# FalkorDB/FalkorDB

Measured on AMD Instinct MI355X. Metric: traversed edges/sec (TEPS) on k-hop MATCH, RMAT scale-22/26; % HBM roofline, higher is better.
Workload: dtype u32

## Files before the change

falkordb_amd/csrc/bitexpand.hip:

```cpp
#include "bitexpand.hpp"

namespace fgpu {

constexpr u32 BP_ITEM = 256;
static_assert(BP_ITEM == 256, "bp_pull_kernel<.., SPARSE> unrolls an item into four 64-entry trips");
constexpr u32 BP_VCHUNK = 4096;

static fgpu_info bp_acc_alloc(fgpu_ctx* ctx, DevBuf<u64>& acc) {
    FGPU_TRY(acc.alloc(ctx, BP_ACC_WORDS));
    FGPU_HIP(hipMemsetAsync(acc.p, 0, BP_ACC_WORDS * sizeof(u64), ctx->stream()));
    return FGPU_OK;
}
__global__ __launch_bounds__(256) void bp_acc_fold_kernel(unsigned long long* __restrict__ acc, u32* __restrict__ pub, u32 seq) {
    __shared__ u64 s_a[4], s_b[4];
    u64 a = acc[(size_t)threadIdx.x * BP_ACC_STRIDE], b = acc[(size_t)threadIdx.x * BP_ACC_STRIDE + 1];
#pragma unroll
    for (int d = 32; d >= 1; d >>= 1) { a += __shfl_xor(a, d, 64); b += __shfl_xor(b, d, 64); }
    if (lane_id() == 0) { s_a[threadIdx.x >> 6] = a; s_b[threadIdx.x >> 6] = b; }
    __syncthreads();
    if (threadIdx.x == 0) {
        const u64 sa = s_a[0] + s_a[1] + s_a[2] + s_a[3], sb = s_b[0] + s_b[1] + s_b[2] + s_b[3];
        if (pub) {
            __hip_atomic_store(pub + 0, (u32)sa, __ATOMIC_RELAXED, __HIP_MEMORY_SCOPE_SYSTEM);
            __hip_atomic_store(pub + 1, (u32)(sa >> 32), __ATOMIC_RELAXED, __HIP_MEMORY_SCOPE_SYSTEM);
// ... 1640 lines not shown
}

static fgpu_info bp_count_finish(fgpu_ctx* ctx, BitState& s, u32 n_out, u32 ntouched, const HopOut& out, u64* nnz, u64* checksum) {
    if (ntouched) {
        ProfScope ps(ctx, "bp_count_kernel<side rows>", (u64)ntouched * s.w * 8);
        DevBuf<u32> vmap;
        FGPU_TRY(vmap.alloc(ctx, (size_t)ntouched + 1));
        FGPU_TRY(launch(bp_slot_vertex_kernel, dim3(ctx->cus * 4), dim3(256), 0, ctx->stream(), out.fin.tbits, out.fin.tpref, n_out, vmap.p));
        FGPU_TRY(bp_count_rows(ctx, s, out.y, ntouched, out.fin.label, out.fin.tab, (u64*)out.fin.acc, 16, vmap.p));
    }
    FGPU_TRY(bp_acc_read(ctx, (u64*)out.fin.acc, nnz, checksum));
    bp_recycle_state(ctx, s);
    s.n = n_out;
    return FGPU_OK;
}

fgpu_info bp_hop(fgpu_ctx* ctx, BitState& s, const fgpu_mat* m, const fgpu_mat* dp, const fgpu_mat* dm, u64* flops,
                 const fgpu_mat* next_m, const fgpu_mat* count_next) {
    HopPlan p;
    FGPU_TRY(bp_hop_enter(ctx, s, m, dp, flops, false));
    FGPU_TRY(bp_hop_plan(ctx, s, m, dp, dm, 0, next_m, count_next, p));
    BitState o;
    bp_layout(o, (u32)m->ncols, s.nsrc);
    FGPU_TRY(bp_alloc_zero(ctx, o.x, o));
    FGPU_TRY(bp_alloc_flags(ctx, o));
    const HopOut out = {o.x.p, o.flag.p, BpFinal{nullptr, nullptr, nullptr, nullptr, nullptr, 0}};
    FusedStats st;
    int pull_idx = -1;
    if (p.t) FGPU_TRY(bp_pull(ctx, p, s, out, next_m, &st, &pull_idx));
    FGPU_TRY(bp_delta_fixups(ctx, p, s, out));
    return bp_hop_finish(ctx, p, s, o, next_m, st, pull_idx);
}

__global__ __launch_bounds__(256) void bp_hub_check_kernel(const u64* __restrict__ x, u32 slot, u32 ws, u32 nsrc, const u32* __restrict__ rowmap,
                                                           const u64* __restrict__ rowhash, u64* __restrict__ out) {
    __shared__ u64 s_h[4];
    bool bad = false;
    for (u32 k = threadIdx.x; k < ws; k += 256) {
        const u32 lo = k * 64;
        const u64 want = nsrc >= lo + 64 ? ~0ull : nsrc > lo ? (1ull << (nsrc - lo)) - 1ull : 0ull;
        bad |= x[(size_t)slot * ws + k] != want;
    }
    u64 hs = 0;
    for (u32 i = threadIdx.x; i < nsrc; i += 256) hs += rowhash ? rowhash[i] : cs_row_hash(rowmap ? (u64)rowmap[i] : (u64)i);
#pragma unroll
    for (int d = 32; d >= 1; d >>= 1) hs += (u64)__shfl_xor((long long)hs, d, 64);
    if (lane_id() == 0) s_h[threadIdx.x >> 6] = hs;
    const int nbad = __syncthreads_count(bad ? 1 : 0);
    if (threadIdx.x == 0) {
        out[0] = nbad == 0 && nsrc ? 1ull : 0ull;
        out[1] = s_h[0] + s_h[1] + s_h[2] + s_h[3];
    }
}
__global__ __launch_bounds__(256) void bp_hub_sums_kernel(const u32* __restrict__ rows, u32 deg, u64 dsum, const u64* __restrict__ label,
                                                          u32 nsrc, const u64* __restrict__ hsum, int with_sum,
                                                          unsigned long long* __restrict__ acc) {
    u64 cnt = 0, ds = 0;
    if (!label) {
        if (blockIdx.x == 0 && threadIdx.x == 0) { cnt = deg; ds = dsum; }
    } else {
        for (u32 i = blockIdx.x * 256 + threadIdx.x; i < deg; i += gridDim.x * 256) {
            const u32 v = rows[i];
            if ((label[v >> 6] >> (v & 63u)) & 1ull) { ++cnt; ds += cs_dest_hash(v); }
        }
    }
    bp_block_add2(cnt * nsrc, with_sum ? ds * hsum[0] : 0ull, acc);
}
static fgpu_info bp_hub_rows(fgpu_ctx* ctx, const BitState& s, const BpXPlan* xp, int mode, const u64* label_dev, u64* acc,
                             const BpXPlan** hub) {
    *hub = nullptr;
    BpXHub hb;
    if (!bp_xplan_hub(xp, &hb) || hb.slot >= s.n || !s.nsrc) return FGPU_OK;
    DevBuf<u64> chk;
    FGPU_TRY(chk.alloc(ctx, 2));
    FGPU_TRY(launch(bp_hub_check_kernel, dim3(1), dim3(256), 0, ctx->stream(), (const u64*)s.x.p, hb.slot, s.ws, s.nsrc,
                    (const u32*)s.rowmap.p, (const u64*)s.rowhash.p, chk.p));
    u32 sat = 0;
    FGPU_TRY(read_u32(ctx, (const u32*)chk.p, &sat));
    if (!sat) return FGPU_OK;
    ProfScope ps(ctx, "xp_hub_rows", (u64)hb.deg * (label_dev ? 4 : 0));
    u32 grid = label_dev ? cdiv(hb.deg, 256) : 1u;
    if (grid > (u32)ctx->cus * 4) grid = ctx->cus * 4;
    FGPU_TRY(launch(bp_hub_sums_kernel, dim3(grid), dim3(256), 0, ctx->stream(), hb.rows, hb.deg, hb.dsum, label_dev, s.nsrc,
                    (const u64*)(chk.p + 1), mode == 2 ? 1 : 0, (unsigned long long*)acc));
    *hub = hb.plan;
    return FGPU_OK;
}

fgpu_info bp_hop_count(fgpu_ctx* ctx, BitState& s, const fgpu_mat* m, const fgpu_mat* dp, const fgpu_mat* dm, u64* flops,
                       const u64* label_dev, u64* nnz, u64* checksum) {
    HopPlan p;
    FGPU_TRY(bp_hop_enter(ctx, s, m, dp, flops, true));
    FGPU_TRY(bp_hop_plan(ctx, s, m, dp, dm, checksum ? 2 : 1, nullptr, nullptr, p));
    FGPU_TRY(bp_relayout(ctx, s, bp_xplan_perm(p.xp)));
    const u32 n_out = (u32)m->ncols;
    DevBuf<u64> tbits, side, tab, acc;
    DevBuf<u32> tpref;
    u32 ntouched = 0;
    if (!p.no_touched) FGPU_TRY(bp_touched_side(ctx, p, s, n_out, tbits, tpref, side, &ntouched));
    FGPU_TRY(bp_acc_alloc(ctx, acc));
    if (p.mode == 2) FGPU_TRY(bp_cs_tables(ctx, s, tab));
    const HopOut out = {side.p, nullptr, BpFinal{tbits.p, tpref.p, label_dev, tab.p, (unsigned long long*)acc.p, s.w}};
    const u64 xrows = s.nz_rows < (u64)s.n ? s.nz_rows : (u64)s.n;
    const BpXPlan* hub = nullptr;
    if (p.no_touched) FGPU_TRY(bp_hub_rows(ctx, s, p.xp, p.mode, label_dev, acc.p, &hub));
    if (p.xp) FGPU_TRY(bp_xpull_count(ctx, hub ? hub : p.xp, p.t, s.x.p, s.ws, p.mode, out.fin, side.p, p.lds_tables, xrows));
    else if (p.t) FGPU_TRY(bp_pull(ctx, p, s, out, nullptr, nullptr, nullptr));
    FGPU_TRY(bp_delta_fixups(ctx, p, s, out));
    return bp_count_finish(ctx, s, n_out, ntouched, out, nnz, checksum);
}

fgpu_info bp_count_hub_in(fgpu_ctx* ctx, const fgpu_mat* m, u32 nsrc, const u64** in_bits) {
    *in_bits = nullptr;
    BitState lay;
    bp_layout(lay, (u32)m->nrows, nsrc);
    if (!m->nnz || m->is_hyper() || !bp_xcd_applies(ctx, lay.n, lay.ws)) return FGPU_OK;
    const fgpu_mat* t = nullptr;
    const BpXPlan* xp = nullptr;
    BpXHub hb;
    FGPU_TRY(transposed_with_items(ctx, m, &t));
    FGPU_TRY(bp_xplan(ctx, m, t, &xp));
    if (bp_xplan_hub(xp, &hb)) *in_bits = hb.in_bits;
    return FGPU_OK;
}

__global__ __launch_bounds__(256) void bp_probe_rows_kernel(CsrView at, const u32* __restrict__ dst, const u32* __restrict__ bit, u32 k,
                                                            const u64* __restrict__ x, u32 ws, uint8_t* __restrict__ hit) {
    const u32 lane = lane_id();
    const u32 wave = (blockIdx.x * 256 + threadIdx.x) >> 6, nwaves = (gridDim.x * 256) >> 6;
    for (u32 i = wave; i < k; i += nwaves) {
        const u32 v = dst[i], j = bit[i];
        if (v == 0xFFFFFFFFu || j == 0xFFFFFFFFu) continue;
        u32 b, e;
        row_range(at, v, b, e);
        bool found = false;
        for (u32 q0 = b; q0 < e && !found; q0 += 64) {
            const u32 q = q0 + lane;
            bool h = false;
            if (q < e) h = (x[(size_t)at.colidx[q] * ws + (j >> 6)] >> (j & 63)) & 1ull;
            found = __ballot(h) != 0ull;
        }
        if (found && lane == 0) hit[i] = 1;
    }
}
__global__ __launch_bounds__(256) void bp_probe_delta_kernel(CsrView d, u32 nnz, const u32* __restrict__ wordrow,
                                                             const u32* __restrict__ sdst, const u32* __restrict__ srow, u32 k,
                                                             const u32* __restrict__ bit, const u64* __restrict__ x, u32 ws,
                                                             uint8_t* __restrict__ hit) {
    for (u32 q = blockIdx.x * 256 + threadIdx.x; q < nnz; q += gridDim.x * 256) {
        const u32 v = d.colidx[q];
        u32 lo = 0, hi = k;
        while (lo < hi) {
            const u32 mid = (lo + hi) >> 1;
            if (sdst[mid] < v) lo = mid + 1; else hi = mid;
        }
// ... 335 lines not shown
```

falkordb_amd/csrc/bitexpand.hpp:

```cpp
#pragma once
#include "common.hpp"

namespace fgpu {

constexpr u32 BP_ACC_SLOTS = 256, BP_ACC_STRIDE = 16;
constexpr size_t BP_ACC_WORDS = (size_t)BP_ACC_SLOTS * BP_ACC_STRIDE;
__device__ __forceinline__ void bp_block_add2(u64 a, u64 b, unsigned long long* __restrict__ acc) {
    __shared__ u64 s_acc_red[32];
#pragma unroll
    for (int d = 32; d >= 1; d >>= 1) {
        a += __shfl_xor(a, d, 64);
        b += __shfl_xor(b, d, 64);
    }
    const u32 wv = threadIdx.x >> 6, nw = (blockDim.x + 63) >> 6;
    if (lane_id() == 0) { s_acc_red[wv] = a; s_acc_red[16 + wv] = b; }
    __syncthreads();
    if (threadIdx.x == 0) {
        u64 sa = 0, sb = 0;
        for (u32 i = 0; i < nw; ++i) { sa += s_acc_red[i]; sb += s_acc_red[16 + i]; }
        unsigned long long* slot = acc + (size_t)(blockIdx.x % BP_ACC_SLOTS) * BP_ACC_STRIDE;
        if (sa) atomicAdd(slot, (unsigned long long)sa);
        if (sb) atomicAdd(slot + 1, (unsigned long long)sb);
    }
}

struct BpFinal {
    const u64* tbits;
    const u32* tpref;
    const u64* label;
    const u64* tab;
    unsigned long long* acc;
    u32 w;
};

struct BpXPlan;
fgpu_info bp_xplan(fgpu_ctx* ctx, const fgpu_mat* m, const fgpu_mat* t, const BpXPlan** out);
fgpu_info bp_xplan_chunks(fgpu_ctx* ctx, const BpXPlan* xp, uint32_t** out, uint64_t* nwords);
const u32* bp_xplan_perm(const BpXPlan* p);
struct BpXHub {
    const BpXPlan* plan;
    u32 slot;
    u32 deg;
    u64 dsum;
    const u32* rows;
    const u64* in_bits;
};
bool bp_xplan_hub(const BpXPlan* xp, BpXHub* out);
fgpu_info bp_xpull_count(fgpu_ctx* ctx, const BpXPlan* xp, const fgpu_mat* t, const u64* x, u32 ws, int mode, const BpFinal& fin,
                         u64* side, size_t lds_tables, u64 xrows);
bool bp_xfold_fits(const fgpu_ctx* ctx, u32 ws, int mode, size_t lds_tables);

}
```

falkordb_amd/csrc/bitpart.hip:

```cpp
#include "bitexpand.hpp"

namespace fgpu {

constexpr u32 XP_FIRST = 0x80000000u;
constexpr u32 XP_SPAN = 768;
constexpr u32 XP_RUNW = 8;
constexpr int XP_FOLD_THREADS = 512;
constexpr u32 XP_RUNS = XP_SPAN / XP_RUNW;
constexpr u32 XP_NO_VTX = 0xFFFFFFFFu;

struct BpXPlan {
    bool usable = false;
    u32 n = 0, ng = 0;
    int cut = 0;
    int dense = 0;
    u32 nd = 0;
    DevBuf<u32> gvtx;
    u64 nentries = 0;
    u32 nprows = 0;
    u32 nchunks = 0;
    DevBuf<u32> pcol;
    u32 pstart[9] = {0, 0, 0, 0, 0, 0, 0, 0, 0};
    u32 cbase[9] = {0, 0, 0, 0, 0, 0, 0, 0, 0};
    DevBuf<u32> pstart_dev;
    DevBuf<u32> cstart;
    DevBuf<u32> crun0;
    DevBuf<uint8_t> cshared;
    DevBuf<u32> zrows;
    u32 nzrows = 0;
    DevBuf<u64> ne;
    DevBuf<u32> pbase;
    int direct = 0;
    u64 ndirect = 0;
    DevBuf<u64> de;
    DevBuf<u32> dbase;
    DevBuf<u32> dcol;
    DevBuf<u32> perm;
    BpXPlanPtr hub;
    u32 hub_v = 0, hub_slot = 0;
    u32 hub_deg = 0;
    u64 hub_dsum = 0;
    DevBuf<u32> hub_rows;
    DevBuf<u64> hub_in;
    const BpXPlan* full = nullptr;
};
const u32* bp_xplan_perm(const BpXPlan* p) { return p ? p->perm.p : nullptr; }
void BpXPlanDelete::operator()(BpXPlan* p) const { delete p; }

__global__ __launch_bounds__(256) void xp_runs_kernel(const uint2* __restrict__ pairs, const u32* __restrict__ pstart, u32 n, u32 nnz,
                                                      u32* __restrict__ pcol, u32* __restrict__ off) {
    __shared__ u32 s_ps[9];
    if (threadIdx.x < 9) s_ps[threadIdx.x] = pstart[threadIdx.x];
    __syncthreads();
    const u32 lane = lane_id();
    const u32 wave = (blockIdx.x * 256 + threadIdx.x) >> 6, nwaves = (gridDim.x * 256) >> 6;
    for (u32 p0 = wave * 64; p0 < nnz; p0 += nwaves * 64) {
        const u32 p = p0 + lane;
        u32 g0 = 0, g1 = 0;
        size_t base = 0;
        if (p < nnz) {
            u32 x = 0;
#pragma unroll
            for (u32 k = 1; k < 8; ++k) x += p >= s_ps[k] ? 1u : 0u;
            const uint2 e = pairs[p];
            const bool head = p == s_ps[x];
            const u32 prev = head ? 0xFFFFFFFFu : pairs[p - 1].y;
            const bool first = head || e.y != prev;
            pcol[p] = e.x | (first ? XP_FIRST : 0u);
            if (first) { g0 = prev + 1u; g1 = e.y + 1u; base = (size_t)x * n; }
        }
        for (int j = 0; j < 2 && g0 < g1; ++j, ++g0) off[base + g0] = p;
        u64 more = __ballot(g0 < g1);
        while (more) {
            const int l = (int)__builtin_ctzll(more);
            more &= more - 1ull;
            const u32 a = (u32)__builtin_amdgcn_readlane((int)g0, l), b = (u32)__builtin_amdgcn_readlane((int)g1, l);
// ... 436 lines not shown
    FGPU_TRY(drop.alloc(ctx, (size_t)n + 1));
    FGPU_HIP(hipMemsetAsync(drop.p, 0, ((size_t)n + 1) * sizeof(u32), st));
    grid = cdiv(deg, 256);
    if (grid > (u32)ctx->cus * 4) grid = ctx->cus * 4;
    FGPU_TRY(launch(xp_hub_rows_kernel, dim3(grid), dim3(256), 0, st, (const u32*)m->rowptr, (const u32*)m->colidx, h, n,
                    (const u32*)t->rowptr, list.p, drop.p, (unsigned long long*)(sums.p + 1)));
    u32 got[4];
    FGPU_TRY(read_words(ctx, (const u32*)(sums.p + 1), 4, got));
    const u64 gone = (u64)got[0] | ((u64)got[1] << 32);
    if (gone * XP_HUB_MIN_SHARE_DEN < t->nnz || gone >= t->nnz) return FGPU_OK;
    FGPU_TRY(kd.alloc(ctx, (size_t)n + 1));
    FGPU_TRY(rp.alloc(ctx, (size_t)n + 1));
    FGPU_TRY(launch(xp_hub_kept_kernel, dim3(ctx->cus * 8), dim3(256), 0, st, (const u32*)t->rowptr, (const u32*)drop.p, n, kd.p));
    FGPU_TRY(scan_u32(ctx, kd.p, rp.p, (u64)n + 1, nullptr));
    u32 kept = 0;
    FGPU_TRY(read_u32(ctx, rp.p + n, &kept));
    FGPU_REQUIRE(kept >= 1 && (u64)kept + gone == t->nnz, FGPU_INVALID, "partitioned pull: the hub's rows hold %llu of %llu entries, %u stay",
                 (unsigned long long)gone, (unsigned long long)t->nnz, kept);
    FGPU_TRY(col.alloc(ctx, kept));
    FGPU_TRY(launch(xp_hub_compact_kernel, dim3(ctx->cus * 16), dim3(256), 0, st, (const u32*)t->rowptr, (const u32*)t->colidx,
                    (const u32*)rp.p, n, col.p));
    const XpSource src = {rp.p, col.p, t->nrows, t->ncols, kept};
    BpXPlanPtr reduced;
    FGPU_TRY(bp_xplan_build(ctx, m, &src, direct, dense, cut, xp, &reduced));
    const size_t nwords = ((size_t)t->ncols + 63) / 64;
    FGPU_TRY(xp->hub_in.alloc(ctx, nwords + 1));
    FGPU_HIP(hipMemsetAsync(xp->hub_in.p, 0, (nwords + 1) * sizeof(u64), st));
    if (h < n) FGPU_TRY(launch(xp_hub_in_kernel, dim3(64), dim3(256), 0, st, (const u32*)t->rowptr, (const u32*)t->colidx, h, xp->hub_in.p));
    u32 slot = h;
    if (xp->perm.p) FGPU_TRY(read_u32(ctx, xp->perm.p + h, &slot));
    FGPU_HIP(hipStreamSynchronize(st));
    xp->hub_v = h; xp->hub_slot = slot; xp->hub_deg = deg;
    xp->hub_dsum = (u64)got[2] | ((u64)got[3] << 32);
    xp->hub_rows = std::move(list);
    reduced->full = xp;
    xp->hub = std::move(reduced);
    return FGPU_OK;
}
bool bp_xplan_hub(const BpXPlan* xp, BpXHub* out) {
    if (!xp || !xp->hub || !xp->hub->usable) return false;
    *out = BpXHub{xp->hub.get(), xp->hub_slot, xp->hub_deg, xp->hub_dsum, xp->hub_rows.p, xp->hub_in.p};
    return true;
}

fgpu_info bp_xplan(fgpu_ctx* ctx, const fgpu_mat* m, const fgpu_mat* t, const BpXPlan** out) {
    *out = nullptr;
    if (!ctx->opt.expand_xcd || !t || t->is_hyper()) return FGPU_OK;
    if (t->ncols >= (1ull << 31) || t->nrows >= 0xFFFFFFC0ull || t->nnz < 4096 || t->nnz >= 0x7FFFFFFFull) return FGPU_OK;
    const int direct = ctx->opt.expand_xp_direct ? 1 : 0, dense = ctx->opt.expand_xp_dense ? 1 : 0, cut = ctx->opt.expand_xp_cut ? 1 : 0;
    std::lock_guard<std::mutex> idx_guard(m->idx_mu);
    BpXPlanPtr& slot = t->bp_xplan[direct + 2 * dense + 4 * cut];
    if (!slot) {
        BpXPlanPtr xp;
        const XpSource src = {t->rowptr, t->colidx, t->nrows, t->ncols, t->nnz};
        if (bp_xplan_build(ctx, m, &src, direct, dense, cut, nullptr, &xp) != FGPU_OK) {
            xp.reset(new (std::nothrow) BpXPlan());
            FGPU_REQUIRE(xp, FGPU_OOM, "out of host memory");
            (void)hipGetLastError();
            set_error("%s", "");
        } else if (bp_xplan_hub_build(ctx, m, t, direct, dense, cut, xp.get()) != FGPU_OK) {
            xp->hub.reset();
            (void)hipStreamSynchronize(ctx->stream());
            (void)hipGetLastError();
            set_error("%s", "");
        }
        slot = std::move(xp);
    }
    if (slot->usable) *out = slot.get();
    return FGPU_OK;
}

fgpu_info bp_xplan_chunks(fgpu_ctx* ctx, const BpXPlan* xp, uint32_t** out, uint64_t* nwords) {
    const size_t nc = xp->nchunks, total = 20 + 3 * nc;
    uint32_t* w = (uint32_t*)ctx->result_alloc(total * sizeof(uint32_t));
    FGPU_REQUIRE(w, FGPU_OOM, "out of host memory");
    w[0] = xp->nchunks; w[1] = (u32)xp->cut;
    for (int k = 0; k <= 8; ++k) { w[2 + k] = xp->pstart[k]; w[11 + k] = xp->cbase[k]; }
    uint32_t* sh = w + 20 + 2 * nc;
    fgpu_info i = nc ? ctx->d2h(w + 20, xp->cstart.p, nc * sizeof(u32)) : FGPU_OK;
    if (i == FGPU_OK && nc) i = ctx->d2h(w + 20 + nc, xp->crun0.p, nc * sizeof(u32));
    if (i == FGPU_OK && nc) i = ctx->d2h(sh, xp->cshared.p, nc);
    if (i != FGPU_OK) { ctx->host_free(w); return i; }
    for (size_t c = nc; c-- > 0;) sh[c] = reinterpret_cast<const uint8_t*>(sh)[c];
    *out = w; *nwords = total;
    return FGPU_OK;
}

__device__ __forceinline__ uint4 or4(uint4 a, uint4 b) { return make_uint4(a.x | b.x, a.y | b.y, a.z | b.z, a.w | b.w); }
__device__ __forceinline__ bool any4(uint4 a) { return (a.x | a.y | a.z | a.w) != 0u; }
__device__ __forceinline__ void atomic_or4(uint4* dst, uint4 v) {
    unsigned long long* d = reinterpret_cast<unsigned long long*>(dst);
    if (v.x | v.y) atomicOr(d, ((unsigned long long)v.y << 32) | v.x);
    if (v.z | v.w) atomicOr(d + 1, ((unsigned long long)v.w << 32) | v.z);
}
// ... 571 lines not shown
```

falkordb_amd/csrc/common.hpp:

```cpp
#pragma once
#include <hip/hip_runtime.h>
#include <stdint.h>
#include <stdlib.h>
#include <string.h>

#include <atomic>
#include <map>
#include <memory>
#include <mutex>
#include <string>
#include <type_traits>
#include <vector>

#include "../../include/fgpu.h"
#include "options.hpp"

namespace fgpu {

typedef uint32_t u32;
typedef uint64_t u64;
typedef int32_t i32;
typedef int64_t i64;

constexpr int WAVE = 64;
// ... 409 lines not shown
                    u64* out_dev, bool zero_out);

struct BitState {
    DevBuf<u64> x;
    u32 n = 0;
    u32 nsrc = 0;
    u32 w = 0;
    u32 ws = 0;
    DevBuf<uint8_t> flag;
    u64 nz_rows = 0;
    const fgpu_mat* pre_for = nullptr;
    u64 pre_flops = 0;
    bool lazy = false;
    const u32* perm = nullptr;
    DevBuf<u32> rowmap;
    DevBuf<u64> rowhash;
    DevBuf<u32> rowrank;
    u32 nsrc_full = 0;
};
fgpu_info bp_from_csr(fgpu_ctx* ctx, BitState& s, const fgpu_mat* f);
fgpu_info bp_push_from_csr(fgpu_ctx* ctx, BitState& s, const fgpu_mat* f, const fgpu_mat* m, const fgpu_mat* dp,
                           const fgpu_mat* dm);
fgpu_info bp_hop(fgpu_ctx* ctx, BitState& s, const fgpu_mat* m, const fgpu_mat* dp, const fgpu_mat* dm, u64* flops,
                 const fgpu_mat* next_m = nullptr, const fgpu_mat* count_next = nullptr);
fgpu_info bp_to_csr(fgpu_ctx* ctx, const BitState& s, const u64* label_dev, fgpu_mat** out);
fgpu_info bp_probe_rows(fgpu_ctx* ctx, const BitState& s, const fgpu_mat* m, const fgpu_mat* dp, const fgpu_mat* dm,
                        const u32* dst_dev, const u32* bit_dev, const u32* sdst_dev, const u32* srow_dev, u32 k,
                        uint8_t* hit_m, uint8_t* hit_dm, uint8_t* hit_dp);
fgpu_info exists_rows(fgpu_ctx* ctx, const fgpu_mat* f, const BitState* s, const fgpu_mat* m, const fgpu_mat* dp, const fgpu_mat* dm,
                      const u64* label_dev, u32 k, u64* sure, u64* maybe, u32 words, u64* entries);
fgpu_info bp_count(fgpu_ctx* ctx, const BitState& s, const u64* label_dev, u64* nnz, u64* checksum);
fgpu_info bp_hop_count(fgpu_ctx* ctx, BitState& s, const fgpu_mat* m, const fgpu_mat* dp, const fgpu_mat* dm, u64* flops,
                       const u64* label_dev, u64* nnz, u64* checksum);
fgpu_info bp_count_hub_in(fgpu_ctx* ctx, const fgpu_mat* m, u32 nsrc, const u64** in_bits);
fgpu_info bp_accumulate(fgpu_ctx* ctx, BitState& u, const BitState& x);
void bp_finish(fgpu_ctx* ctx, BitState& s);

constexpr u32 HUB_DEG = 4096;
constexpr u32 HUB_CHUNK = 4096;
constexpr u32 PUSH_HUB_DEG = 1024;
constexpr u32 PUSH_HUB_CHUNK = 1024;

}
```

falkordb_amd/csrc/spgemm.hip:

```cpp
#include <algorithm>
#include <string>
#include <thread>

#include "common.hpp"

namespace fgpu {

__global__ void entry_deg_kernel(CsrView f, CsrView b, u32 nnzf, u32* __restrict__ deg) {
    u32 e = blockIdx.x * blockDim.x + threadIdx.x;
    if (e >= nnzf) { if (e == nnzf) deg[e] = 0; return; }
    u32 s = f.colidx[e], rb, re;
    row_range(b, s, rb, re);
    deg[e] = re - rb;
}

__global__ void gather_u64_kernel(const u64* __restrict__ eoff, const u32* __restrict__ frp, u32 k,
                                  u64* __restrict__ roff, u32* __restrict__ maxlen) {
    u32 i = blockIdx.x * blockDim.x + threadIdx.x;
    if (i > k) return;
    roff[i] = eoff[frp[i]];
    if (i < k) {
        u32 len = frp[i + 1] - frp[i];
        u32 m = len;
#pragma unroll
// ... 1147 lines not shown
    const u32 m = cnt[i];
    const u32 n = scan_class_rows_of(k, key[i], m, kmax);
    if (!n) return;
    u64 h;
    if (key[i] == SCAN_NOKEY) h = cs_row_hash(lrow[i]);
    else {
        const u32 low = (u32)__ffs(m) - 1;
        h = (k == (low < kmax ? low : kmax)) ? hsum[i] : 0ull;
    }
    const u32 p = pos[(u64)k * nlive + i];
    for (u32 q = 0; q < n && p + q < nrows; ++q) {
        rid[p + q] = lid[i];
        rrow[p + q] = lrow[i];
        rhash[p + q] = q ? 0ull : h;
    }
}

__global__ void scan_strong_kernel(const u32* __restrict__ lid, u32 nlive, CsrView m0, const u64* __restrict__ in_h, u32 nbits,
                                   u32* __restrict__ weak) {
    const u32 i = blockIdx.x * blockDim.x + threadIdx.x;
    if (i > nlive) return;
    u32 w = 0;
    if (i < nlive) {
        u32 b, e;
        row_range(m0, lid[i], b, e);
        w = 1;
        for (u32 q = b; q < e && w; ++q) {
            const u32 t = m0.colidx[q];
            if (t < nbits && ((in_h[t >> 6] >> (t & 63u)) & 1ull)) w = 0;
        }
    }
    weak[i] = w;
}
__global__ void scan_strong_move_kernel(const u32* __restrict__ lid, const u32* __restrict__ lrow, const u32* __restrict__ weak,
                                        const u32* __restrict__ wpos, u32 nlive, u32* __restrict__ olid, u32* __restrict__ olrow) {
    const u32 i = blockIdx.x * blockDim.x + threadIdx.x;
    if (i >= nlive) return;
    const u32 p = weak[i] ? nlive - wpos[nlive] + wpos[i] : i - wpos[i];
    olid[p] = lid[i];
    olrow[p] = lrow[i];
}
static fgpu_info scan_strong_first(fgpu_ctx* ctx, const Layers& L, DevBuf<u32>& lid, DevBuf<u32>& lrow, u32 nlive, u32 pass_rows) {
    if (L.nhops != 3 || L.m[1] != L.m[2] || L.m[0]->ncols != L.m[1]->nrows) return FGPU_OK;
    for (int h = 0; h < 3; ++h)
        if ((L.dp_at(h) && L.dp_at(h)->nnz) || (L.dm_at(h) && L.dm_at(h)->nnz)) return FGPU_OK;
    const u64* in_h = nullptr;
    FGPU_TRY(bp_count_hub_in(ctx, L.m[2], pass_rows, &in_h));
    if (!in_h) return FGPU_OK;
    ProfScope ps(ctx, "scan strong first", 0);
    DevBuf<u32> weak, wpos, olid, olrow;
    FGPU_TRY(weak.alloc(ctx, (size_t)nlive + 1));
    FGPU_TRY(wpos.alloc(ctx, (size_t)nlive + 1));
    FGPU_TRY(olid.alloc(ctx, nlive));
    FGPU_TRY(olrow.alloc(ctx, nlive));
    FGPU_TRY(launch(scan_strong_kernel, dim3(cdiv((u64)nlive + 1, 256)), dim3(256), 0, ctx->stream(), (const u32*)lid.p, nlive,
                    view_of(L.m[0]), in_h, (u32)L.m[1]->nrows, weak.p));
    FGPU_TRY(scan_u32(ctx, weak.p, wpos.p, (u64)nlive + 1, nullptr));
    FGPU_TRY(launch(scan_strong_move_kernel, dim3(cdiv(nlive, 256)), dim3(256), 0, ctx->stream(), (const u32*)lid.p, (const u32*)lrow.p,
                    (const u32*)weak.p, (const u32*)wpos.p, nlive, olid.p, olrow.p));
    lid = std::move(olid);
    lrow = std::move(olrow);
    return FGPU_OK;
}

struct ScanPass { u32 first, rows, scale; };

static void scan_cut_passes(const u32* rows, u32 groups, u32 pass_rows, std::vector<ScanPass>& out) {
    u32 first = 0;
    for (u32 g = 0; g < groups; ++g) {
        for (u32 o = 0; o < rows[g]; o += pass_rows) out.push_back({first + o, std::min(pass_rows, rows[g] - o), 1u << g});
        first += rows[g];
    }
}

struct ScanClasses {
    DevBuf<u32> rid, rrow;
    DevBuf<u64> rhash;
    u32 kmax = 0;
    u32 rows[SCAN_KMAX + 1] = {};
};
static fgpu_info scan_build_classes(fgpu_ctx* ctx, const fgpu_mat* m0, const u32* lid, const u32* lrow, u32 nlive, u32 pass_rows,
                                    ScanClasses& sc) {
    ProfScope ps(ctx, "scan classes", 0);
    DevBuf<u32> key, rep, cnt, stats;
    DevBuf<u64> hsum;
    const u32 grid = cdiv(nlive, 256);
    FGPU_TRY(key.alloc(ctx, nlive));
    FGPU_TRY(cnt.alloc(ctx, nlive));
    FGPU_TRY(hsum.alloc(ctx, nlive));
    FGPU_TRY(rep.alloc(ctx, m0->ncols));
    FGPU_TRY(stats.alloc(ctx, 2 * (SCAN_KMAX + 1)));
    FGPU_HIP(hipMemsetAsync(rep.p, 0xFF, (size_t)m0->ncols * sizeof(u32), ctx->stream()));
// ... 763 lines not shown
```

Measured before the change: 15190 billion.

## Extend hub shortcut to a set of top-degree hubs with tiered scan ordering

Builds a second reduced pull plan that removes the rows adjacent to up to 32 top-degree hubs, not only the single top hub. When every hub slot is saturated, their contributions are counted in closed form. A per-vertex hub bitmask lets the 3-hop scan sort sources into three tiers (all hubs reached, some, top hub missing), so passes that saturate every hub can use the smaller plan. This adds build-time preprocessing, a larger check kernel and extra scans in exchange for skipping more edge work in the count path.

```diff
diff --git a/falkordb_amd/csrc/bitexpand.hip b/falkordb_amd/csrc/bitexpand.hip
--- a/falkordb_amd/csrc/bitexpand.hip
+++ b/falkordb_amd/csrc/bitexpand.hip
@@ -1696,29 +1696,43 @@
     return bp_hop_finish(ctx, p, s, o, next_m, st, pull_idx);
 }
 
-__global__ __launch_bounds__(256) void bp_hub_check_kernel(const u64* __restrict__ x, u32 slot, u32 ws, u32 nsrc, const u32* __restrict__ rowmap,
-                                                           const u64* __restrict__ rowhash, u64* __restrict__ out) {
+__global__ __launch_bounds__(256) void bp_hub_check_kernel(const u64* __restrict__ x, u32 n, u32 slot, const u32* __restrict__ slots, u32 nh,
+                                                           u32 ws, u32 nsrc, const u32* __restrict__ rowmap, const u64* __restrict__ rowhash,
+                                                           u64* __restrict__ out) {
     __shared__ u64 s_h[4];
-    bool bad = false;
-    for (u32 k = threadIdx.x; k < ws; k += 256) {
-        const u32 lo = k * 64;
+    __shared__ u32 s_bad[2];
+    if (threadIdx.x < 2) s_bad[threadIdx.x] = 0u;
+    __syncthreads();
+    if (!slots) nh = 1;
+    bool bad1 = false, bad2 = false;
+    for (u32 k = threadIdx.x; k < nh * ws; k += 256) {
+        const u32 i = k / ws, wd = k - i * ws;
+        const u32 r = i ? slots[i] : slot;
+        const u32 lo = wd * 64;
         const u64 want = nsrc >= lo + 64 ? ~0ull : nsrc > lo ? (1ull << (nsrc - lo)) - 1ull : 0ull;
-        bad |= x[(size_t)slot * ws + k] != want;
+        const bool bad = r >= n || x[(size_t)r * ws + wd] != want;
+        if (i) bad2 |= bad;
+        else bad1 |= bad;
     }
     u64 hs = 0;
     for (u32 i = threadIdx.x; i < nsrc; i += 256) hs += rowhash ? rowhash[i] : cs_row_hash(rowmap ? (u64)rowmap[i] : (u64)i);
 #pragma unroll
     for (int d = 32; d >= 1; d >>= 1) hs += (u64)__shfl_xor((long long)hs, d, 64);
     if (lane_id() == 0) s_h[threadIdx.x >> 6] = hs;
-    const int nbad = __syncthreads_count(bad ? 1 : 0);
+    if (bad1) s_bad[0] = 1u;
+    if (bad2) s_bad[1] = 1u;
+    __syncthreads();
     if (threadIdx.x == 0) {
-        out[0] = nbad == 0 && nsrc ? 1ull : 0ull;
+        const u32 level = s_bad[0] || !nsrc ? 0u : (nh >= 2 && !s_bad[1]) ? 2u : 1u;
+        out[0] = level;
         out[1] = s_h[0] + s_h[1] + s_h[2] + s_h[3];
     }
 }
+template <int LEVEL>
 __global__ __launch_bounds__(256) void bp_hub_sums_kernel(const u32* __restrict__ rows, u32 deg, u64 dsum, const u64* __restrict__ label,
                                                           u32 nsrc, const u64* __restrict__ hsum, int with_sum,
                                                           unsigned long long* __restrict__ acc) {
+    static_assert(LEVEL == 1 || LEVEL == 2, "one reduced plan, or two");
     u64 cnt = 0, ds = 0;
     if (!label) {
         if (blockIdx.x == 0 && threadIdx.x == 0) { cnt = deg; ds = dsum; }
@@ -1737,17 +1751,28 @@
     if (!bp_xplan_hub(xp, &hb) || hb.slot >= s.n || !s.nsrc) return FGPU_OK;
     DevBuf<u64> chk;
     FGPU_TRY(chk.alloc(ctx, 2));
-    FGPU_TRY(launch(bp_hub_check_kernel, dim3(1), dim3(256), 0, ctx->stream(), (const u64*)s.x.p, hb.slot, s.ws, s.nsrc,
-                    (const u32*)s.rowmap.p, (const u64*)s.rowhash.p, chk.p));
-    u32 sat = 0;
-    FGPU_TRY(read_u32(ctx, (const u32*)chk.p, &sat));
-    if (!sat) return FGPU_OK;
-    ProfScope ps(ctx, "xp_hub_rows", (u64)hb.deg * (label_dev ? 4 : 0));
-    u32 grid = label_dev ? cdiv(hb.deg, 256) : 1u;
+    FGPU_TRY(launch(bp_hub_check_kernel, dim3(1), dim3(256), 0, ctx->stream(), (const u64*)s.x.p, s.n, hb.slot,
+                    hb.set_plan ? hb.set_slots : nullptr, hb.set_plan ? hb.set_n : 1u, s.ws, s.nsrc, (const u32*)s.rowmap.p,
+                    (const u64*)s.rowhash.p, chk.p));
+    u32 level = 0;
+    FGPU_TRY(read_u32(ctx, (const u32*)chk.p, &level));
+    if (!level) return FGPU_OK;
+    const bool set = level >= 2 && hb.set_plan;
+    const u32 deg = set ? hb.set_deg : hb.deg;
+    ProfScope ps(ctx, "xp_hub_rows", (u64)deg * (label_dev ? 4 : 0));
+    u32 grid = label_dev ? cdiv(deg, 256) : 1u;
     if (grid > (u32)ctx->cus * 4) grid = ctx->cus * 4;
-    FGPU_TRY(launch(bp_hub_sums_kernel, dim3(grid), dim3(256), 0, ctx->stream(), hb.rows, hb.deg, hb.dsum, label_dev, s.nsrc,
-                    (const u64*)(chk.p + 1), mode == 2 ? 1 : 0, (unsigned long long*)acc));
-    *hub = hb.plan;
+    const u64* hsum = chk.p + 1;
+    const int with_sum = mode == 2 ? 1 : 0;
+    if (set) {
+        ProfScope ps2(ctx, "xp_hub_set", 0);
+        FGPU_TRY(launch(bp_hub_sums_kernel<2>, dim3(grid), dim3(256), 0, ctx->stream(), hb.set_rows, deg, hb.set_dsum, label_dev, s.nsrc,
+                        hsum, with_sum, (unsigned long long*)acc));
+    } else {
+        FGPU_TRY(launch(bp_hub_sums_kernel<1>, dim3(grid), dim3(256), 0, ctx->stream(), hb.rows, deg, hb.dsum, label_dev, s.nsrc, hsum,
+                        with_sum, (unsigned long long*)acc));
+    }
+    *hub = set ? hb.set_plan : hb.plan;
     return FGPU_OK;
 }
 
@@ -1774,8 +1799,10 @@
     return bp_count_finish(ctx, s, n_out, ntouched, out, nnz, checksum);
 }
 
-fgpu_info bp_count_hub_in(fgpu_ctx* ctx, const fgpu_mat* m, u32 nsrc, const u64** in_bits) {
+fgpu_info bp_count_hub_in(fgpu_ctx* ctx, const fgpu_mat* m, u32 nsrc, const u64** in_bits, const u32** hub_mask, u32* set_n) {
     *in_bits = nullptr;
+    *hub_mask = nullptr;
+    *set_n = 0;
     BitState lay;
     bp_layout(lay, (u32)m->nrows, nsrc);
     if (!m->nnz || m->is_hyper() || !bp_xcd_applies(ctx, lay.n, lay.ws)) return FGPU_OK;
@@ -1784,7 +1811,10 @@
     BpXHub hb;
     FGPU_TRY(transposed_with_items(ctx, m, &t));
     FGPU_TRY(bp_xplan(ctx, m, t, &xp));
-    if (bp_xplan_hub(xp, &hb)) *in_bits = hb.in_bits;
+    if (bp_xplan_hub(xp, &hb)) {
+        *in_bits = hb.in_bits;
+        if (hb.set_plan) { *hub_mask = hb.hub_mask; *set_n = hb.set_n; }
+    }
     return FGPU_OK;
 }
 
diff --git a/falkordb_amd/csrc/bitexpand.hpp b/falkordb_amd/csrc/bitexpand.hpp
--- a/falkordb_amd/csrc/bitexpand.hpp
+++ b/falkordb_amd/csrc/bitexpand.hpp
@@ -44,6 +44,13 @@
     u64 dsum;
     const u32* rows;
     const u64* in_bits;
+    const BpXPlan* set_plan = nullptr;
+    u32 set_n = 0;
+    const u32* set_slots = nullptr;
+    u32 set_deg = 0;
+    u64 set_dsum = 0;
+    const u32* set_rows = nullptr;
+    const u32* hub_mask = nullptr;
 };
 bool bp_xplan_hub(const BpXPlan* xp, BpXHub* out);
 fgpu_info bp_xpull_count(fgpu_ctx* ctx, const BpXPlan* xp, const fgpu_mat* t, const u64* x, u32 ws, int mode, const BpFinal& fin,
diff --git a/falkordb_amd/csrc/bitpart.hip b/falkordb_amd/csrc/bitpart.hip
--- a/falkordb_amd/csrc/bitpart.hip
+++ b/falkordb_amd/csrc/bitpart.hip
@@ -1,3 +1,5 @@
+#include <algorithm>
+
 #include "bitexpand.hpp"
 
 namespace fgpu {
@@ -42,6 +44,15 @@
     u64 hub_dsum = 0;
     DevBuf<u32> hub_rows;
     DevBuf<u64> hub_in;
+    u64 hub_gone = 0;
+    BpXPlanPtr hub2;
+    u32 hset_n = 0;
+    u32 hset_v[32] = {};
+    DevBuf<u32> hset_slots;
+    u32 hset_deg = 0;
+    u64 hset_dsum = 0;
+    DevBuf<u32> hset_rows;
+    DevBuf<u32> hub_mask;
     const BpXPlan* full = nullptr;
 };
 const u32* bp_xplan_perm(const BpXPlan* p) { return p ? p->perm.p : nullptr; }
@@ -544,14 +555,171 @@
     FGPU_HIP(hipStreamSynchronize(st));
     xp->hub_v = h; xp->hub_slot = slot; xp->hub_deg = deg;
     xp->hub_dsum = (u64)got[2] | ((u64)got[3] << 32);
+    xp->hub_gone = gone;
     xp->hub_rows = std::move(list);
     reduced->full = xp;
     xp->hub = std::move(reduced);
     return FGPU_OK;
 }
+
+constexpr u32 XP_HUB_SET_DEG_DEN = 4;
+constexpr u32 XP_HUB_SET_MAX = 32;
+constexpr u32 XP_HUB_SET_MIN_SHARE_DEN = 8;
+constexpr u32 XP_HUB_SET_LIST = 1024;
+static_assert(XP_HUB_SET_MAX == 32, "hub_mask is a u32 per vertex, BpXPlan::hset_v holds 32");
+__global__ __launch_bounds__(256) void xp_hub_set_list_kernel(const u32* __restrict__ rowptr, u32 nrows, u32 mindeg, u32 cap,
+                                                              u64* __restrict__ keys, u32* __restrict__ cnt) {
+    for (u32 u = blockIdx.x * 256 + threadIdx.x; u < nrows; u += gridDim.x * 256) {
+        const u32 d = rowptr[u + 1] - rowptr[u];
+        if (d >= mindeg) {
+            const u32 i = atomicAdd(cnt, 1u);
+            if (i < cap) keys[i] = ((u64)d << 32) | (u64)(~u);
+        }
+    }
+}
+__global__ __launch_bounds__(256) void xp_hub_set_rows_kernel(const u32* __restrict__ mrowptr, const u32* __restrict__ mcol,
+                                                              const u32* __restrict__ hs, u32 n, u32* __restrict__ drop) {
+    const u32 h = hs[blockIdx.y];
+    const u32 b = mrowptr[h], deg = mrowptr[h + 1] - b;
+    for (u32 i = blockIdx.x * 256 + threadIdx.x; i < deg; i += gridDim.x * 256) {
+        const u32 v = mcol[b + i];
+        if (v < n) drop[v] = 1u;
+    }
+}
+__global__ __launch_bounds__(256) void xp_hub_set_sums_kernel(const u32* __restrict__ trowptr, const u32* __restrict__ drop, u32 n,
+                                                              unsigned long long* __restrict__ sums) {
+    u64 ent = 0, ds = 0;
+    for (u32 v = blockIdx.x * 256 + threadIdx.x; v < n; v += gridDim.x * 256)
+        if (drop[v]) {
+            ent += trowptr[v + 1] - trowptr[v];
+            ds += cs_dest_hash(v);
+        }
+#pragma unroll
+    for (int d = 32; d >= 1; d >>= 1) {
+        ent += (u64)__shfl_xor((long long)ent, d, 64);
+        ds += (u64)__shfl_xor((long long)ds, d, 64);
+    }
+    if (lane_id() == 0) {
+        if (ent) atomicAdd(sums, (unsigned long long)ent);
+        if (ds) atomicAdd(sums + 1, (unsigned long long)ds);
+    }
+}
+__global__ void xp_hub_set_compact_kernel(const u32* __restrict__ drop, const u32* __restrict__ pos, u32 n, u32* __restrict__ list) {
+    for (u32 v = blockIdx.x * 256 + threadIdx.x; v < n; v += gridDim.x * 256)
+        if (drop[v]) list[pos[v]] = v;
+}
+__global__ __launch_bounds__(256) void xp_hub_set_mask_kernel(const u32* __restrict__ trowptr, const u32* __restrict__ tcol,
+                                                              const u32* __restrict__ hs, u32 n, u32 ncols, u32* __restrict__ mask) {
+    const u32 h = hs[blockIdx.y];
+    if (h >= n) return;
+    const u32 b = trowptr[h], e = trowptr[h + 1];
+    for (u32 q = b + blockIdx.x * 256 + threadIdx.x; q < e; q += gridDim.x * 256) {
+        const u32 u = tcol[q];
+        if (u < ncols) atomicOr(&mask[u], 1u << blockIdx.y);
+    }
+}
+__global__ void xp_hub_set_slots_kernel(const u32* __restrict__ hs, const u32* __restrict__ perm, u32 nh, u32* __restrict__ slots) {
+    if (threadIdx.x < nh) slots[threadIdx.x] = perm ? perm[hs[threadIdx.x]] : hs[threadIdx.x];
+}
+
+static fgpu_info bp_xplan_hub_set_build(fgpu_ctx* ctx, const fgpu_mat* m, const fgpu_mat* t, int direct, int dense, int cut, BpXPlan* xp) {
+    if (!xp->hub || !xp->hub->usable || !xp->hub_deg) return FGPU_OK;
+    hipStream_t st = ctx->stream();
+    const u32 n = (u32)t->nrows, nu = (u32)m->nrows;
+    const u32 mindeg = cdiv(xp->hub_deg, XP_HUB_SET_DEG_DEN);
+    DevBuf<u64> keys;
+    DevBuf<u32> cnt;
+    FGPU_TRY(cnt.alloc(ctx, 1));
+    u32 grid = cdiv(nu, 256);
+    if (grid > (u32)ctx->cus * 8) grid = ctx->cus * 8;
+    u32 cap = XP_HUB_SET_LIST, found = 0;
+    for (int round = 0; round < 2; ++round) {
+        FGPU_TRY(keys.alloc(ctx, cap));
+        FGPU_HIP(hipMemsetAsync(cnt.p, 0, sizeof(u32), st));
+        FGPU_TRY(launch(xp_hub_set_list_kernel, dim3(grid), dim3(256), 0, st, (const u32*)m->rowptr, nu, mindeg, cap, keys.p, cnt.p));
+        FGPU_TRY(read_u32(ctx, cnt.p, &found));
+        if (found <= cap) break;
+        cap = found;
+    }
+    if (found < 2 || found > cap) return FGPU_OK;
+    std::vector<u64> hk(found);
+    FGPU_TRY(ctx->d2h(hk.data(), keys.p, (size_t)found * sizeof(u64)));
+    std::sort(hk.begin(), hk.end(), [](u64 a, u64 b) { return a > b; });
+    const u32 nh = found < XP_HUB_SET_MAX ? found : XP_HUB_SET_MAX;
+    u32 hv[XP_HUB_SET_MAX] = {};
+    for (u32 i = 0; i < nh; ++i) hv[i] = ~(u32)hk[i];
+    if (hv[0] != xp->hub_v) return FGPU_OK;
+    DevBuf<u32> hs, drop, pos, list, kd, rp, col, slots, mask;
+    DevBuf<u64> sums;
+    FGPU_TRY(hs.alloc(ctx, XP_HUB_SET_MAX));
+    FGPU_TRY(ctx->h2d(hs.p, hv, sizeof(hv)));
+    FGPU_TRY(drop.alloc(ctx, (size_t)n + 1));
+    FGPU_HIP(hipMemsetAsync(drop.p, 0, ((size_t)n + 1) * sizeof(u32), st));
+    FGPU_TRY(sums.alloc(ctx, 2));
+    FGPU_HIP(hipMemsetAsync(sums.p, 0, 2 * sizeof(u64), st));
+    grid = cdiv(xp->hub_deg, 256);
+    if (grid > (u32)ctx->cus * 4) grid = ctx->cus * 4;
+    FGPU_TRY(launch(xp_hub_set_rows_kernel, dim3(grid, nh), dim3(256), 0, st, (const u32*)m->rowptr, (const u32*)m->colidx,
+                    (const u32*)hs.p, n, drop.p));
+    FGPU_TRY(launch(xp_hub_set_sums_kernel, dim3(ctx->cus * 8), dim3(256), 0, st, (const u32*)t->rowptr, (const u32*)drop.p, n,
+                    (unsigned long long*)sums.p));
+    u32 got[4];
+    FGPU_TRY(read_words(ctx, (const u32*)sums.p, 4, got));
+    const u64 gone = (u64)got[0] | ((u64)got[1] << 32);
+    if (gone < xp->hub_gone || gone >= t->nnz) return FGPU_OK;
+    if ((gone - xp->hub_gone) * XP_HUB_SET_MIN_SHARE_DEN < t->nnz) return FGPU_OK;
+    FGPU_TRY(pos.alloc(ctx, (size_t)n + 1));
+    FGPU_TRY(scan_u32(ctx, drop.p, pos.p, (u64)n + 1, nullptr));
+    u32 nrows_u = 0;
+    FGPU_TRY(read_u32(ctx, pos.p + n, &nrows_u));
+    FGPU_REQUIRE(nrows_u >= xp->hub_deg && nrows_u <= n, FGPU_INVALID, "partitioned pull: the hub set's union holds %u rows, the top hub's %u",
+                 nrows_u, xp->hub_deg);
+    FGPU_TRY(list.alloc(ctx, nrows_u));
+    FGPU_TRY(launch(xp_hub_set_compact_kernel, dim3(ctx->cus * 8), dim3(256), 0, st, (const u32*)drop.p, (const u32*)pos.p, n, list.p));
+    FGPU_TRY(kd.alloc(ctx, (size_t)n + 1));
+    FGPU_TRY(rp.alloc(ctx, (size_t)n + 1));
+    FGPU_TRY(launch(xp_hub_kept_kernel, dim3(ctx->cus * 8), dim3(256), 0, st, (const u32*)t->rowptr, (const u32*)drop.p, n, kd.p));
+    FGPU_TRY(scan_u32(ctx, kd.p, rp.p, (u64)n + 1, nullptr));
+    u32 kept = 0;
+    FGPU_TRY(read_u32(ctx, rp.p + n, &kept));
+    FGPU_REQUIRE(kept >= 1 && (u64)kept + gone == t->nnz, FGPU_INVALID, "partitioned pull: the hub set's rows hold %llu of %llu entries, %u stay",
+                 (unsigned long long)gone, (unsigned long long)t->nnz, kept);
+    FGPU_TRY(col.alloc(ctx, kept));
+    FGPU_TRY(launch(xp_hub_compact_kernel, dim3(ctx->cus * 16), dim3(256), 0, st, (const u32*)t->rowptr, (const u32*)t->colidx,
+                    (const u32*)rp.p, n, col.p));
+    const XpSource src = {rp.p, col.p, t->nrows, t->ncols, kept};
+    BpXPlanPtr reduced;
+    FGPU_TRY(bp_xplan_build(ctx, m, &src, direct, dense, cut, xp, &reduced));
+    FGPU_TRY(mask.alloc(ctx, (size_t)t->ncols + 1));
+    FGPU_HIP(hipMemsetAsync(mask.p, 0, ((size_t)t->ncols + 1) * sizeof(u32), st));
+    FGPU_TRY(launch(xp_hub_set_mask_kernel, dim3(64, nh), dim3(256), 0, st, (const u32*)t->rowptr, (const u32*)t->colidx,
+                    (const u32*)hs.p, n, (u32)t->ncols, mask.p));
+    FGPU_TRY(slots.alloc(ctx, XP_HUB_SET_MAX));
+    FGPU_TRY(launch(xp_hub_set_slots_kernel, dim3(1), dim3(64), 0, st, (const u32*)hs.p, (const u32*)xp->perm.p, nh, slots.p));
+    FGPU_HIP(hipStreamSynchronize(st));
+    xp->hset_n = nh;
+    memcpy(xp->hset_v, hv, sizeof(hv));
+    xp->hset_slots = std::move(slots);
+    xp->hset_deg = nrows_u;
+    xp->hset_dsum = (u64)got[2] | ((u64)got[3] << 32);
+    xp->hset_rows = std::move(list);
+    xp->hub_mask = std::move(mask);
+    reduced->full = xp;
+    xp->hub2 = std::move(reduced);
+    return FGPU_OK;
+}
 bool bp_xplan_hub(const BpXPlan* xp, BpXHub* out) {
     if (!xp || !xp->hub || !xp->hub->usable) return false;
     *out = BpXHub{xp->hub.get(), xp->hub_slot, xp->hub_deg, xp->hub_dsum, xp->hub_rows.p, xp->hub_in.p};
+    if (xp->hub2 && xp->hub2->usable) {
+        out->set_plan = xp->hub2.get();
+        out->set_n = xp->hset_n;
+        out->set_slots = xp->hset_slots.p;
+        out->set_deg = xp->hset_deg;
+        out->set_dsum = xp->hset_dsum;
+        out->set_rows = xp->hset_rows.p;
+        out->hub_mask = xp->hub_mask.p;
+    }
     return true;
 }
 
@@ -572,6 +740,11 @@
             set_error("%s", "");
         } else if (bp_xplan_hub_build(ctx, m, t, direct, dense, cut, xp.get()) != FGPU_OK) {
             xp->hub.reset();
+            (void)hipStreamSynchronize(ctx->stream());
+            (void)hipGetLastError();
+            set_error("%s", "");
+        } else if (bp_xplan_hub_set_build(ctx, m, t, direct, dense, cut, xp.get()) != FGPU_OK) {
+            xp->hub2.reset();
             (void)hipStreamSynchronize(ctx->stream());
             (void)hipGetLastError();
             set_error("%s", "");
diff --git a/falkordb_amd/csrc/common.hpp b/falkordb_amd/csrc/common.hpp
--- a/falkordb_amd/csrc/common.hpp
+++ b/falkordb_amd/csrc/common.hpp
@@ -465,7 +465,7 @@
 fgpu_info bp_count(fgpu_ctx* ctx, const BitState& s, const u64* label_dev, u64* nnz, u64* checksum);
 fgpu_info bp_hop_count(fgpu_ctx* ctx, BitState& s, const fgpu_mat* m, const fgpu_mat* dp, const fgpu_mat* dm, u64* flops,
                        const u64* label_dev, u64* nnz, u64* checksum);
-fgpu_info bp_count_hub_in(fgpu_ctx* ctx, const fgpu_mat* m, u32 nsrc, const u64** in_bits);
+fgpu_info bp_count_hub_in(fgpu_ctx* ctx, const fgpu_mat* m, u32 nsrc, const u64** in_bits, const u32** hub_mask, u32* set_n);
 fgpu_info bp_accumulate(fgpu_ctx* ctx, BitState& u, const BitState& x);
 void bp_finish(fgpu_ctx* ctx, BitState& s);
 
diff --git a/falkordb_amd/csrc/spgemm.hip b/falkordb_amd/csrc/spgemm.hip
--- a/falkordb_amd/csrc/spgemm.hip
+++ b/falkordb_amd/csrc/spgemm.hip
@@ -1203,11 +1203,32 @@
     }
     weak[i] = w;
 }
+__global__ void scan_tier_kernel(const u32* __restrict__ lid, u32 nlive, CsrView m0, const u32* __restrict__ mask, u32 nbits, u32 all,
+                                 u32* __restrict__ mid, u32* __restrict__ weak) {
+    const u32 i = blockIdx.x * blockDim.x + threadIdx.x;
+    if (i > nlive) return;
+    u32 got = all;
+    if (i < nlive) {
+        u32 b, e;
+        row_range(m0, lid[i], b, e);
+        got = 0;
+        for (u32 q = b; q < e && got != all; ++q) {
+            const u32 t = m0.colidx[q];
+            if (t < nbits) got |= mask[t] & all;
+        }
+    }
+    mid[i] = (got & 1u) && got != all ? 1u : 0u;
+    weak[i] = (got & 1u) ? 0u : 1u;
+}
 __global__ void scan_strong_move_kernel(const u32* __restrict__ lid, const u32* __restrict__ lrow, const u32* __restrict__ weak,
-                                        const u32* __restrict__ wpos, u32 nlive, u32* __restrict__ olid, u32* __restrict__ olrow) {
+                                        const u32* __restrict__ wpos, const u32* __restrict__ mid, const u32* __restrict__ mpos,
+                                        u32 nlive, u32* __restrict__ olid, u32* __restrict__ olrow) {
     const u32 i = blockIdx.x * blockDim.x + threadIdx.x;
     if (i >= nlive) return;
-    const u32 p = weak[i] ? nlive - wpos[nlive] + wpos[i] : i - wpos[i];
+    const u32 nweak = wpos[nlive], nmid = mid ? mpos[nlive] : 0u, mbefore = mid ? mpos[i] : 0u;
+    const u32 p = weak[i]               ? nlive - nweak + wpos[i]
+                  : (mid && mid[i])     ? nlive - nweak - nmid + mbefore
+                                        : i - wpos[i] - mbefore;
     olid[p] = lid[i];
     olrow[p] = lrow[i];
 }
@@ -1216,19 +1237,30 @@
     for (int h = 0; h < 3; ++h)
         if ((L.dp_at(h) && L.dp_at(h)->nnz) || (L.dm_at(h) && L.dm_at(h)->nnz)) return FGPU_OK;
     const u64* in_h = nullptr;
-    FGPU_TRY(bp_count_hub_in(ctx, L.m[2], pass_rows, &in_h));
+    const u32* mask = nullptr;
+    u32 nh = 0;
+    FGPU_TRY(bp_count_hub_in(ctx, L.m[2], pass_rows, &in_h, &mask, &nh));
     if (!in_h) return FGPU_OK;
     ProfScope ps(ctx, "scan strong first", 0);
-    DevBuf<u32> weak, wpos, olid, olrow;
+    DevBuf<u32> weak, wpos, mid, mpos, olid, olrow;
     FGPU_TRY(weak.alloc(ctx, (size_t)nlive + 1));
     FGPU_TRY(wpos.alloc(ctx, (size_t)nlive + 1));
     FGPU_TRY(olid.alloc(ctx, nlive));
     FGPU_TRY(olrow.alloc(ctx, nlive));
-    FGPU_TRY(launch(scan_strong_kernel, dim3(cdiv((u64)nlive + 1, 256)), dim3(256), 0, ctx->stream(), (const u32*)lid.p, nlive,
-                    view_of(L.m[0]), in_h, (u32)L.m[1]->nrows, weak.p));
+    if (mask && nh >= 2) {
+        FGPU_TRY(mid.alloc(ctx, (size_t)nlive + 1));
+        FGPU_TRY(mpos.alloc(ctx, (size_t)nlive + 1));
+        const u32 all = nh >= 32 ? 0xFFFFFFFFu : (1u << nh) - 1u;
+        FGPU_TRY(launch(scan_tier_kernel, dim3(cdiv((u64)nlive + 1, 256)), dim3(256), 0, ctx->stream(), (const u32*)lid.p, nlive,
+                        view_of(L.m[0]), mask, (u32)L.m[1]->nrows, all, mid.p, weak.p));
+        FGPU_TRY(scan_u32(ctx, mid.p, mpos.p, (u64)nlive + 1, nullptr));
+    } else {
+        FGPU_TRY(launch(scan_strong_kernel, dim3(cdiv((u64)nlive + 1, 256)), dim3(256), 0, ctx->stream(), (const u32*)lid.p, nlive,
+                        view_of(L.m[0]), in_h, (u32)L.m[1]->nrows, weak.p));
+    }
     FGPU_TRY(scan_u32(ctx, weak.p, wpos.p, (u64)nlive + 1, nullptr));
     FGPU_TRY(launch(scan_strong_move_kernel, dim3(cdiv(nlive, 256)), dim3(256), 0, ctx->stream(), (const u32*)lid.p, (const u32*)lrow.p,
-                    (const u32*)weak.p, (const u32*)wpos.p, nlive, olid.p, olrow.p));
+                    (const u32*)weak.p, (const u32*)wpos.p, (const u32*)mid.p, (const u32*)mpos.p, nlive, olid.p, olrow.p));
     lid = std::move(olid);
     lrow = std::move(olrow);
     return FGPU_OK;
```

Result: faster. 18070 billion (median of 6 runs) (+18.9%).
